# arhix52/Strelka

Measured on AMD Instinct MI355X. Metric: Mray/s, higher is better.
Workload: dtype f32; 1 GPU; kitchen stand-in (SURVEY 8d C3): 1724134 unique triangles, 2022 instances of 153 meshes, 4 rect + 1 distant light, 60/25/10/5 % diffuse/glossy/metal/glass; resolution=1920x1080, bounces=4, spp=64, tile=32, world_size=1, parallelism=single GPU, rays_per_frame=839862650

## Files before the change

### strelka_amd/build.py

```python
import os
import subprocess

HERE = os.path.dirname(os.path.abspath(__file__))
ROOT = os.path.dirname(HERE)
LIB = os.environ.get("SKH_LIB") or os.path.join(HERE, "libstrelka_hip.so")
SRC = os.path.join(HERE, "csrc", "strelka_hip.hip")
DEPS = [SRC] + [os.path.join(HERE, "csrc", f) for f in ("skh_device.h", "skh_bvh.h", "skh_env.h", "skh_emit.h", "skh_blend.h", "skh_lshape.h", "skh_kernels.h", "skh_shade_body.inc", "skh_trace_body.inc", "skh_libm.h", "skh_host.h", "skh_accel.inc")] + [
    os.path.join(ROOT, "include", "strelka_hip.h"), os.path.abspath(__file__)]
FLAGS = ["-O3", "--offload-arch=gfx950", "-ffp-contract=off", "-fno-slp-vectorize", "-mllvm", "-amdgpu-sched-strategy=max-ilp",
         "-fPIC", "-shared", "-std=c++17"]


def hipcc():
    for c in (os.environ.get("HIPCC"), "/opt/rocm/bin/hipcc", "hipcc"):
        if c and (os.path.isabs(c) and os.path.exists(c) or not os.path.isabs(c)):
            return c
    return "hipcc"


def needs_build():
    if os.environ.get("SKH_LIB") and os.path.exists(LIB):
        return False
    return not os.path.exists(LIB) or any(os.path.getmtime(d) > os.path.getmtime(LIB) for d in DEPS)


def build_variant(out_path, defines, verbose=False):
    cmd = [hipcc()] + FLAGS + ["-D" + d for d in defines] + ["-o", out_path, SRC]
    if verbose:
        print(" ".join(cmd))
    subprocess.check_call(cmd)
    return out_path


def build(force=False, verbose=False):
    if not force and not needs_build():
        return LIB
    import fcntl

    with open(LIB + ".lock", "w") as lock:
        fcntl.flock(lock, fcntl.LOCK_EX)
# ... 60 lines not shown
```

### strelka_amd/csrc/skh_host.h

```cpp
#pragma once
#include "../../include/strelka_hip.h"
#include "skh_kernels.h"

#include <string>
#include <utility>
#include <vector>

typedef struct ncclComm* ncclComm_t;
using namespace skh;

namespace
{
struct DevBuf
{
    void* p = nullptr;
    size_t bytes = 0;
    DevBuf() = default;
    DevBuf(const DevBuf&) = delete;
    DevBuf& operator=(const DevBuf&) = delete;
    DevBuf(DevBuf&& o) noexcept : p(o.p), bytes(o.bytes)
    {
        o.p = nullptr;
        o.bytes = 0;
    }
    DevBuf& operator=(DevBuf&& o) noexcept
    {
        if (this != &o)
        {
            reset();
            p = o.p, bytes = o.bytes;
            o.p = nullptr, o.bytes = 0;
        }
        return *this;
    }
    ~DevBuf()
// ... 139 lines not shown
    uint32_t width = 0, height = 0, tileSize = 32, tileShift = 5, numTiles = 0, numSlots = 0;
    std::vector<uint32_t> tileXY;
    bool customTiles = false;
    DevBuf dTileXY, dAccum, dDiffuse, dSpecular, dDiffCnt, dSpecCnt, dSums, dPath, dRayQ[2], dHits, dShadowQ, dContrib, dCounts,
        dOvf, dOvf2, dStats, dScratchImage;
    uint32_t traceBlocks = 0;
    uint32_t curveSplitBuilt = 1;
    uint32_t numWorldCurves = 0;
    int worldCurveRoot[SKH_WORLD_CURVES];
    uint32_t worldCurveInst[SKH_WORLD_CURVES];
    uint32_t worldCurveMerged = 0;
    uint32_t worldCurveIdentLast = 0;
    uint32_t hierNodes = 0;
    int32_t fetchChunk = -1;
    uint32_t numTlasLeaves = 0;
    bool countTraversal = false, timing = false;
    uint32_t wavesPerCU = 28;
    uint32_t wavesPerCUShadow = 28;
    uint32_t wavesPerCUShadowWorld = 32;
    uint32_t queueConstBits[2] = { 0, 0 };
    bool queueConstFilled = false;
    uint32_t reinsertRounds = 8;
    uint32_t reinsertCurveRounds = 4;
    uint32_t reinsertMinSize = 0;
    skh_build_info buildInfo = {};
    uint32_t plocTop = 0;
    uint32_t wavesPerCUWorld = 32;
    uint32_t smallWavesClosest = 0, smallWavesShadow = 0;
    uint32_t gridOverride = 0;
    uint32_t fetchMinClosestSmall = 48;
    bool fetchMinClosestSet = false;
    uint32_t smallWavesFirst = 0, smallWavesLast = 0;
    int tailSplit = 1;
    bool splitNow = false;
    uint32_t fetchMinClosest = 32 , fetchMinShadow = 48;
    uint32_t curveFetchMinClosest = 16, curveFetchMinShadow = 16 , curveNodeBreakClosest = 20, curveNodeBreakShadow = 20;
    uint32_t nodeBreakClosest = 32, nodeBreakShadow = 28;
    uint32_t worldCurveMin = 32;
    uint32_t curveMin = 48;
    uint32_t leafMin = 16;
    uint32_t subframeBatch = 0, batchCapacity = 1;
    uint32_t queueRegion = 64;
    bool tightInstanceBoxes = true;
    uint32_t curveLeaf = 1;
    uint32_t numMergedCurveInst = 0;
    uint32_t splitPairs = 0;
    uint32_t curveMerge = 1;
    uint32_t curveSegNode = 0;
    uint32_t curveStrandMajor = 0;
    uint32_t curveSplit = 4;
    uint32_t tlasBuild = 1;
    uint32_t tlasOpen = 1;
    uint32_t bakeWorld = 4, bakeSmallTris = 64, bakeBudgetMTris = 64;
    bool worldKernel = true;
    std::vector<uint8_t> baked;
    int worldRoot = SKH_REF_INVALID, lightRoot = SKH_REF_INVALID;
    uint32_t nBakedTris = 0, nBakedInst = 0;
    uint32_t mortonBits = 10;
    uint32_t leafLines = 0;
    uint32_t nTriSlots = 0;
    LightBox lightBox = { { -INFINITY, -INFINITY, -INFINITY }, { INFINITY, INFINITY, INFINITY } };
    uint32_t mergeLightProxies = 0;
    uint32_t nShadeRecords = 0;
    int32_t directRecordsOpt = -1;
    uint32_t directRecords = 1;
    uint32_t hitPrimRange = 0;
// ... 54 lines not shown
```

### strelka_amd/csrc/skh_kernels.h

```cpp
#pragma once
#include "skh_bvh.h"
#include "skh_env.h"
#include "skh_emit.h"
#include "skh_blend.h"

namespace skh
{

struct DevInstance
{
    float w2o[12];
    int rootRef;
    uint32_t mask;
    uint32_t type;
    uint32_t pad;
};
struct HostInstance
{
    float o2w[12];
    uint32_t type, geom, material, light;
};

#define SKH_WORLD_CURVES 2
#define SKH_SEG_STRIDE 8
// ... 119 lines not shown
    return mk3(rcp_safe(d.x), rcp_safe(d.y), rcp_safe(d.z));
}
#define SKH_SLAB_SLACK 1.0000019073486328125f

struct TraceCounters
{
    uint32_t nodes, prims, segs, insts;
};

SKH_DI bool slab_test(const v3& lo, const v3& hi, const v3& o, const v3& inv, float tmin, float tmax, float& tnear)
{
    const float t0x = (lo.x - o.x) * inv.x, t1x = (hi.x - o.x) * inv.x;
    const float t0y = (lo.y - o.y) * inv.y, t1y = (hi.y - o.y) * inv.y;
    const float t0z = (lo.z - o.z) * inv.z, t1z = (hi.z - o.z) * inv.z;
    const float tn = fmaxf(fmaxf(fminf(t0x, t1x), fminf(t0y, t1y)), fmaxf(fminf(t0z, t1z), tmin));
    const float tf = fminf(fminf(fmaxf(t0x, t1x), fmaxf(t0y, t1y)), fminf(fmaxf(t0z, t1z), tmax));
    tnear = tn;
    return tn <= tf * 1.0000002384185791015625f;
}

struct HitRec
{
    float t;
    uint32_t inst, prim;
    float u, v;
    bool found;
};

struct StatsDev
{
    unsigned long long raysRadiance, raysShadow, nodes[2], prims[2], segs[2], insts[2];
#ifdef SKH_LANE_PROFILE
    unsigned long long wave[2][10];
    unsigned long long shade[8];
    unsigned int slowCount, slowPad;
    float slow[16][12];
    unsigned long long runHist[2][42], blockHist[2][42];
    unsigned long long cyc[2][10];
#endif
#ifdef SKH_TAIL_PROFILE
    unsigned long long launchT0[2], dryHist[2][64], exitHist[2][64], afterDryHist[2][64], dryLive[2][65], rayTicksAfterDry[2], waveTicksAfterDry[2];
#endif
};

SKH_DI uint32_t rank_below(unsigned long long mask)
{
    return __builtin_amdgcn_mbcnt_hi((uint32_t)(mask >> 32), __builtin_amdgcn_mbcnt_lo((uint32_t)mask, 0u));
}
SKH_DI uint32_t wave_max(uint32_t v)
{
#pragma unroll
    for (int off = 32; off >= 1; off >>= 1)
        v = max(v, (uint32_t)__shfl_xor(v, off));
    return v;
}

SKH_DI uint32_t wave_sum(uint32_t v)
{
#pragma unroll
    for (int off = 32; off >= 1; off >>= 1)
        v += __shfl_xor(v, off);
    return v;
}

#ifndef SKH_CURVE_MIN_WAVES
#define SKH_CURVE_MIN_WAVES 6
#endif
// ... 611 lines not shown
    if (i >= n)
        return;
    const uint32_t mid0 = material[i] == 0xffffffffu ? 0u : material[i], mid = mid0 < numMaterials ? mid0 : 0u;
    Material mat = materials[mid];
    const float4 l = Le[mid];
    v3 le = mk3(l.x, l.y, l.z);
    resolve_material(texels, texDesc, numTextures, mat, mtex_entry(mt, mid), le, uv[2 * (size_t)i], uv[2 * (size_t)i + 1]);
    float* o = out + 8 * (size_t)i;
    o[0] = mat.base_color[0], o[1] = mat.base_color[1], o[2] = mat.base_color[2], o[3] = mat.roughness, o[4] = mat.metallic;
    o[5] = le.x, o[6] = le.y, o[7] = le.z;
}
__global__ void __launch_bounds__(256) k_emit_probe_mtex(EmitP em, MtexP mt, DevScene sc, const float* __restrict__ in, uint32_t n, uint32_t* __restrict__ out)
{
    const uint32_t i = blockIdx.x * blockDim.x + threadIdx.x;
    if (i >= n)
        return;
    const float* q = in + 6 * (size_t)i;
    const EmitSample s = emit_sample(em, q[0], q[1], q[2], mk3(q[3], q[4], q[5]));
    const v3 Le = s.Le * emit_sample_texel(mt, sc, s.instance, s.prim, q[1], q[2]);
    uint32_t* o = out + 13 * (size_t)i;
    o[0] = __float_as_uint(s.point.x), o[1] = __float_as_uint(s.point.y), o[2] = __float_as_uint(s.point.z);
    o[3] = __float_as_uint(s.normal.x), o[4] = __float_as_uint(s.normal.y), o[5] = __float_as_uint(s.normal.z);
    o[6] = __float_as_uint(Le.x), o[7] = __float_as_uint(Le.y), o[8] = __float_as_uint(Le.z);
    o[9] = __float_as_uint(s.pdf), o[10] = __float_as_uint(s.dist), o[11] = s.instance, o[12] = s.prim;
}

#ifndef SKH_SHADE_WAVES
#define SKH_SHADE_WAVES(HAIR) ((HAIR) ? 4 : 5)
#endif
#define SKH_SHADE_ATTR(HAIR) __attribute__((amdgpu_waves_per_eu(SKH_SHADE_WAVES(HAIR), SKH_SHADE_WAVES(HAIR))))
#ifndef SKH_SHADE_BLOCK
#define SKH_SHADE_BLOCK 256
#endif
template <bool HAIR, bool ENV, bool EMIT, bool MTEX>
__global__ void __launch_bounds__(SKH_SHADE_BLOCK) SKH_SHADE_ATTR(HAIR)
    k_shade(DevScene sc, FrameP fp, uint32_t sampleOffset, uint32_t depth , const uint32_t* __restrict__ tileXY, RayQ rq,
            const uint32_t* __restrict__ countPtr, HitQ hq, PathS ps, RayQ nextQ, uint32_t* __restrict__ nextCount, RayQ shadowQ,
            float4* __restrict__ contrib, uint32_t* __restrict__ shadowCount, EnvP env, EmitP emit, MtexP mtex)
{
    constexpr bool LSHAPE = false;
    const LshapeP lsh = { nullptr };
#include "skh_shade_body.inc"
}
template <bool HAIR, bool ENV, bool EMIT, bool MTEX>
__global__ void __launch_bounds__(SKH_SHADE_BLOCK) SKH_SHADE_ATTR(HAIR)
    k_shade_lshape(DevScene sc, FrameP fp, uint32_t sampleOffset, uint32_t depth , const uint32_t* __restrict__ tileXY, RayQ rq,
                   const uint32_t* __restrict__ countPtr, HitQ hq, PathS ps, RayQ nextQ, uint32_t* __restrict__ nextCount, RayQ shadowQ,
                   float4* __restrict__ contrib, uint32_t* __restrict__ shadowCount, EnvP env, EmitP emit, MtexP mtex, LshapeP lsh)
{
    constexpr bool LSHAPE = true;
#include "skh_shade_body.inc"
}

__global__ void __launch_bounds__(256) k_lshape_probe(const Light* __restrict__ lights, uint32_t numLights, LshapeP lsh, uint32_t rectMethod, uint32_t kind,
                                                      const uint32_t* __restrict__ in, uint32_t n, float* __restrict__ out)
{
    const uint32_t i = blockIdx.x * blockDim.x + threadIdx.x;
    if (i >= n)
        return;
    const uint32_t* q = in + (kind == 0u ? 6u : 7u) * (size_t)i;
    const uint32_t lid = q[0];
    float* o = out + (kind == 0u ? 13u : 2u) * (size_t)i;
    if (lid >= numLights)
    {
        for (uint32_t k = 0; k < (kind == 0u ? 13u : 2u); ++k)
            o[k] = 0.0f;
        return;
    }
    const Light light = lights[lid];
    Lshape lse;
    lse.flags = 0u, lse.cosOuter = lse.cosInner = lse.focus = 0.0f, lse.axis = mk3(0.0f);
    if (lsh.table)
        lse = lshape_fetch(lsh, lid);
    const bool sampledDisc = light.type == 1 && (lse.flags & SKH_LSHAPE_SAMPLE_DISC) != 0u;
    if (kind == 0u)
    {
        const float ux = __uint_as_float(q[1]), uy = __uint_as_float(q[2]);
        const v3 P = mk3(__uint_as_float(q[3]), __uint_as_float(q[4]), __uint_as_float(q[5]));
        LightSample d;
        d.pointOnLight = mk3(0.0f), d.pdf = 0.0f, d.normal = mk3(0.0f), d.area = 0.0f, d.L = mk3(0.0f), d.distToLight = 0.0f;
        switch (light.type)
// ... 682 lines not shown
```

### strelka_amd/csrc/skh_shade_body.inc

```
    const uint32_t numPick = (ENV ? sc.numLights + (env.nee ? 1u : 0u) : sc.numLights) + (EMIT ? (emit.nee ? 1u : 0u) : 0u);
    __shared__ uint32_t s_wave[2 * (SKH_COMPACT_MAX_WAVES + 1)];
    __shared__ uint32_t s_sobol[SKH_SOBOL_LUT_WORDS];
#if SKH_MATERIALS_LDS
    __shared__ float4 s_mat[SKH_MATERIALS_LDS * 4];
#endif
    const uint32_t shard = blockIdx.x & (SKH_SHARDS - 1u), lb = blockIdx.x / SKH_SHARDS;
    const uint32_t n = countPtr[shard * SKH_COUNT_STRIDE];
    if (lb * blockDim.x >= n)
        return;
    const uint32_t il = lb * blockDim.x + threadIdx.x;
    const uint32_t i = shard * rq.region + il;
#ifdef SKH_LANE_PROFILE
    unsigned long long spc[8] = { 0, 0, 0, 0, 0, 0, 0, 0 }, spT = __builtin_readcyclecounter();
#define SKH_SP(k)                                                    \
    {                                                                \
        const unsigned long long t_ = __builtin_readcyclecounter();  \
        spc[k] += t_ - spT;                                          \
        spT = t_;                                                    \
    }
#else
#define SKH_SP(k)
#endif
    bool valid = il < n;
    uint32_t pid = 0;
    v3 rayO = mk3(0.0f), rayD = mk3(0.0f);
    float4 hr0 = make_float4(0.0f, 0.0f, 0.0f, 0.0f), hr1 = hr0;
    {
        constexpr int passes = ((SKH_SOBOL_LUT_WORDS / 4) + SKH_SHADE_BLOCK - 1) / SKH_SHADE_BLOCK;
        uint4 lut[passes];
#pragma unroll
        for (int k = 0; k < passes; ++k)
            if ((k + 1) * SKH_SHADE_BLOCK <= SKH_SOBOL_LUT_WORDS / 4 || threadIdx.x + k * SKH_SHADE_BLOCK < SKH_SOBOL_LUT_WORDS / 4)
                lut[k] = reinterpret_cast<const uint4*>(g_sobol_lut)[threadIdx.x + k * SKH_SHADE_BLOCK];
            else
                lut[k] = make_uint4(0u, 0u, 0u, 0u);
#if SKH_MATERIALS_LDS
        float4 mrow = make_float4(0.0f, 0.0f, 0.0f, 0.0f);
        static_assert(SKH_MATERIALS_LDS * 4 <= SKH_SHADE_BLOCK, "one float4 of the material table per thread");
        if (threadIdx.x < SKH_MATERIALS_LDS * 4 && threadIdx.x < sc.numMaterials * 4u)
            mrow = reinterpret_cast<const float4*>(sc.materials)[threadIdx.x];
#endif
#pragma unroll
        for (int k = 0; k < passes; ++k)
            if ((k + 1) * SKH_SHADE_BLOCK <= SKH_SOBOL_LUT_WORDS / 4 || threadIdx.x + k * SKH_SHADE_BLOCK < SKH_SOBOL_LUT_WORDS / 4)
                reinterpret_cast<uint4*>(s_sobol)[threadIdx.x + k * SKH_SHADE_BLOCK] = lut[k];
#if SKH_MATERIALS_LDS
        if (threadIdx.x < SKH_MATERIALS_LDS * 4)
            s_mat[threadIdx.x] = mrow;
#endif
    }
    __syncthreads();
    bool emitNext = false, emitShadow = false;
    v3 nextO = mk3(0.0f), nextD = mk3(0.0f), shO = mk3(0.0f), shD = mk3(0.0f), shC = mk3(0.0f);
    float shTmax = 0.0f;
    if (valid)
    {
        pid = rq.ids()[i];
        rayO = mk3(rq.plane(0)[i], rq.plane(1)[i], rq.plane(2)[i]);
        rayD = mk3(rq.plane(3)[i], rq.plane(4)[i], rq.plane(5)[i]);
        if (hq.primBits != 0u)
        {
            hr0 = *hq.rec16(i);
            const uint32_t w = __float_as_uint(hr0.w);
            hr1.x = __uint_as_float(w == 0xffffffffu ? w : w >> hq.primBits);
            hr1.y = __uint_as_float(w == 0xffffffffu ? w : ((w & ((1u << hq.primBits) - 1u)) | (hq.direct ? SKH_PRIM_DIRECT : 0u)));
        }
        else
            hr0 = hq.rec(i)[0], hr1 = hq.rec(i)[1];
        const float ht = hr0.x, hu = hr0.y, hv = hr0.z;
        const uint32_t hinst = __float_as_uint(hr1.x), hprim = __float_as_uint(hr1.y);
        float* P = ps.base;
        const size_t S = ps.stride;
        v3 throughput = depth == 0u ? mk3(1.0f) : mk3(P[pid], P[pid + S], P[pid + 2 * S]);
        v3 radiance = mk3(0.0f);
        bool radianceDirty = false;
#define SKH_RADIANCE_LOAD() radiance = mk3(ps.rad()[pid]), radianceDirty = true
        float lastBsdfPdf = depth == 0u ? 0.0f : P[pid + 6 * S];
        uint32_t flags = depth == 0u ? 0u : reinterpret_cast<uint32_t*>(P)[pid + 7 * S];
        bool inside = (flags & PF_INSIDE) != 0;
        bool specularBounce = (flags & PF_SPECULAR) != 0;
        uint32_t firstEvent = (flags >> PF_EVENT_SHIFT) & 3u;
        uint32_t px, py;
        const uint32_t sub = pid / fp.numSlots;
        slot_to_pixel(fp, tileXY, pid - sub * fp.numSlots, px, py);
        Sampler smp = init_sampler(px, py, fp.subframeIndex + sampleOffset + sub, fp.sppTotal, 52u);
        smp.depth = depth;
        uint32_t prdDepth = depth;
        v3 origin = rayO, dir = rayD;

        if (hinst == 0xffffffffu)
        {
            if constexpr (ENV)
            {
                const EnvEval ee = env_eval(env, rayD);
                SKH_RADIANCE_LOAD();
                if (depth == 0 || specularBounce || !env.nee)
                    radiance = radiance + throughput * ee.Le;
                else
                {
                    const float lightPdf = ee.pdf / (float)numPick;
                    const float misWeight = mis_weight_balance(lastBsdfPdf, lightPdf);
// ... 366 lines not shown
        {
            const float p = fmaxf(throughput.x, fmaxf(throughput.y, throughput.z));
            if (sampler_random_lut(smp, DIM_RR, s_sobol) > p)
                alive = false;
            else
                throughput = throughput * (1.0f / (p + 1e-5f));
        }
        if (alive && dot(throughput, throughput) < 1e-5f)
            alive = false;
        if (alive)
        {
            ++prdDepth;
            if (fp.debug == 1)
                alive = false;
        }
        if (alive && prdDepth >= fp.maxDepth)
            alive = false;
        emitNext = alive;
        nextO = origin;
        nextD = dir;
        P[pid] = throughput.x;
        P[pid + S] = throughput.y;
        P[pid + 2 * S] = throughput.z;
        if (radianceDirty)
        {
            ps.rad()[pid] = make_float4(radiance.x, radiance.y, radiance.z, 0.0f);
        }
#undef SKH_RADIANCE_LOAD
        P[pid + 6 * S] = lastBsdfPdf;
        reinterpret_cast<uint32_t*>(P)[pid + 7 * S] =
            (inside ? PF_INSIDE : 0u) | (specularBounce ? PF_SPECULAR : 0u) | (firstEvent << PF_EVENT_SHIFT);
    }
    SKH_SP(6)
    uint32_t ni, si;
    block_compact2(emitNext, nextCount + shard * SKH_COUNT_STRIDE, emitShadow, shadowCount + shard * SKH_COUNT_STRIDE, s_wave, ni, si);
    ni += shard * nextQ.region;
    si += shard * shadowQ.region;
    if (emitNext)
    {
        nextQ.plane(0)[ni] = nextO.x;
        nextQ.plane(1)[ni] = nextO.y;
        nextQ.plane(2)[ni] = nextO.z;
        nextQ.plane(3)[ni] = nextD.x;
        nextQ.plane(4)[ni] = nextD.y;
        nextQ.plane(5)[ni] = nextD.z;
        nextQ.ids()[ni] = pid;
    }
    if (emitShadow)
    {
        shadowQ.plane(0)[si] = shO.x;
        shadowQ.plane(1)[si] = shO.y;
        shadowQ.plane(2)[si] = shO.z;
        shadowQ.plane(3)[si] = shD.x;
        shadowQ.plane(4)[si] = shD.y;
        shadowQ.plane(5)[si] = shD.z;
        shadowQ.plane(7)[si] = shTmax;
        contrib[si] = make_float4(shC.x, shC.y, shC.z, __uint_as_float(pid));
    }
#ifdef SKH_LANE_PROFILE
    SKH_SP(7)
    for (int k = 0; k < 8; ++k)
    {
        const uint32_t hi32 = wave_max((uint32_t)(spc[k] >> 4));
        if ((threadIdx.x & 63u) == 0)
            atomicAdd(&sc.profile->shade[k], (unsigned long long)hi32 << 4);
    }
#endif
#undef SKH_SP
```

### strelka_amd/csrc/strelka_hip.hip

```cpp
#include "../../include/strelka_hip.h"
#include "skh_kernels.h"

#include <dlfcn.h>
typedef struct ncclComm* ncclComm_t;
typedef struct
{
    char internal[128];
} ncclUniqueId;
typedef enum
{
    ncclSuccess = 0
} ncclResult_t;
typedef enum
{
    ncclFloat = 7
} ncclDataType_t;

#include <algorithm>
#include <chrono>
#include <cmath>
#include <cstdio>
#include <cstring>
#include <mutex>
#include <string>
// ... 1600 lines not shown
    const bool oneSampleDirect = batch == 1 && fp.samplesThisLaunch == 1 && finalize && fp.finalFirst == 0 && fp.finalCount == 1;
    for (uint32_t s = 0; trace && s < fp.samplesThisLaunch; ++s)
    {
        SKH_TRY(c, hipMemsetAsync(counts, 0, sizeof(uint32_t) * (QW * 2 * SKH_MAX_LAUNCH_ROUNDS + 16 * SKH_FETCH_STRIDE * (rounds + 1) + (size_t)(cutOn ? rounds : 0u) * cutBounceWords), st));
        blp.sampleBase = fp.subframeIndex + s;
        {
            SpanGuard g(c, KC_RAYGEN);
            k_raygen<<<c->raygenBlocksPerSub * fp.batch, 512, 0, st>>>(fp, tiles, s, rq[0], counts, ps, c->dRaygenBase.as<uint32_t>(),
                                                                       c->raygenBlocksPerSub, c->raygenValidPerSub);
        }
        for (uint32_t b = 0; b < rounds; ++b)
        {
            {
                SpanGuard g(c, KC_TRACE_CLOSEST);
                c->gridOverride = (useOverlap && smallPass) ? ((b == 0 && c->smallWavesFirst) ? c->smallWavesFirst : c->smallWavesClosest ? c->smallWavesClosest : (c->nSegs ? 16u : 20u)) * (uint32_t)c->numCUs : 0u;
                if (c->countTraversal)
                    launch_trace<false, true>(c, sc, rq[b & 1], counts + 2 * b * QW, fetch + 16 * b * SKH_FETCH_STRIDE, hq, ps, nullptr);
                else
                    launch_trace<false, false>(c, sc, rq[b & 1], counts + 2 * b * QW, fetch + 16 * b * SKH_FETCH_STRIDE, hq, ps, nullptr);
                if (cutOn)
                {
                    blp.depth = b;
                    if (c->countTraversal)
                        run_cutout_chain<false, true>(c, sc, sc, rq[b & 1], counts + 2 * b * QW, hq, hq, nullptr, ps, nullptr, cutQ[0], cutQ[1], cutH, cutWords + (size_t)b * cutBounceWords, NP, st, blp);
                    else
                        run_cutout_chain<false, false>(c, sc, sc, rq[b & 1], counts + 2 * b * QW, hq, hq, nullptr, ps, nullptr, cutQ[0], cutQ[1], cutH, cutWords + (size_t)b * cutBounceWords, NP, st, blp);
                }
            }
            if (useOverlap && b > 0)
                (void)hipStreamWaitEvent(st, c->evShadow, 0);
            {
                SpanGuard g(c, KC_SHADE);
                const uint32_t perShard = (((NP + SKH_SHARDS - 1u) / SKH_SHARDS) + 63u) & ~63u;
                const dim3 sg(SKH_SHARDS * ((perShard + SKH_SHADE_BLOCK - 1) / SKH_SHADE_BLOCK));
#define SKH_SHADE_LAUNCH_MTEX(HAIRB, ENVB, EMITB, MTEXB)                                                                                                                             \
    if (lshp.table)                                                                                                                                                                  \
        k_shade_lshape<HAIRB, ENVB, EMITB, MTEXB><<<sg, SKH_SHADE_BLOCK, 0, st>>>(sc, fp, s, b, tiles, rq[b & 1], counts + 2 * b * QW, hq, ps, rq[(b + 1) & 1],                       \
                                                                                  counts + 2 * (b + 1) * QW, shq, c->dContrib.as<float4>(), counts + (2 * b + 1) * QW, envp, emitp,  \
                                                                                  mtexp, lshp);                                                                                      \
    else                                                                                                                                                                             \
        k_shade<HAIRB, ENVB, EMITB, MTEXB><<<sg, SKH_SHADE_BLOCK, 0, st>>>(sc, fp, s, b, tiles, rq[b & 1], counts + 2 * b * QW, hq, ps, rq[(b + 1) & 1], counts + 2 * (b + 1) * QW, \
                                                                           shq, c->dContrib.as<float4>(), counts + (2 * b + 1) * QW, envp, emitp, mtexp)
#define SKH_SHADE_LAUNCH(HAIRB, ENVB, EMITB)              \
    if (mtexp.count)                                      \
    {                                                     \
        SKH_SHADE_LAUNCH_MTEX(HAIRB, ENVB, EMITB, true);  \
    }                                                     \
    else                                                  \
    {                                                     \
        SKH_SHADE_LAUNCH_MTEX(HAIRB, ENVB, EMITB, false); \
    }
#define SKH_SHADE_LAUNCH_EMIT(HAIRB, ENVB)     \
    if (emitp.count)                           \
    {                                          \
        SKH_SHADE_LAUNCH(HAIRB, ENVB, true);   \
    }                                          \
    else                                       \
    {                                          \
        SKH_SHADE_LAUNCH(HAIRB, ENVB, false);  \
    }
                if (c->hasHairMaterial && c->envW)
                {
                    SKH_SHADE_LAUNCH_EMIT(true, true);
                }
                else if (c->hasHairMaterial)
                {
                    SKH_SHADE_LAUNCH_EMIT(true, false);
                }
                else if (c->envW)
                {
                    SKH_SHADE_LAUNCH_EMIT(false, true);
                }
                else
                {
                    SKH_SHADE_LAUNCH_EMIT(false, false);
// ... 1082 lines not shown
struct OptRow
{
    const char* name;
    int64_t lo, hi;
    OptEffect effect;
    void (*store)(skh_context*, int64_t);
    bool needsSegNode = false;
    bool skh_context::*counters = nullptr;
};
static const int64_t kOptMin = INT64_MIN, kOptMax = INT64_MAX;
#define OPT_U32(field) [](skh_context* c, int64_t v) { c->field = (uint32_t)v; }
#define OPT_I32(field) [](skh_context* c, int64_t v) { c->field = (int32_t)v; }
#define OPT_FLAG(field) [](skh_context* c, int64_t v) { c->field = v != 0; }
static const OptRow kOptions[] = {
    { "count_traversal", kOptMin, kOptMax, OPT_NONE, OPT_FLAG(countTraversal), false, &skh_context::countTraversal },
    { "timing", kOptMin, kOptMax, OPT_NONE, OPT_FLAG(timing), false, &skh_context::timing },
    { "fetch_min_closest", 1, 64, OPT_NONE, [](skh_context* c, int64_t v) { c->fetchMinClosestSet = true, c->fetchMinClosest = c->curveFetchMinClosest = (uint32_t)v; } },
    { "fetch_min_shadow", 1, 64, OPT_NONE, [](skh_context* c, int64_t v) { c->fetchMinShadow = c->curveFetchMinShadow = (uint32_t)v; } },
    { "node_break_closest", 0, 64, OPT_NONE, [](skh_context* c, int64_t v) { c->nodeBreakClosest = c->curveNodeBreakClosest = (uint32_t)v; } },
    { "node_break_shadow", 0, 64, OPT_NONE, [](skh_context* c, int64_t v) { c->nodeBreakShadow = c->curveNodeBreakShadow = (uint32_t)v; } },
    { "curve_min", 1, 64, OPT_NONE, [](skh_context* c, int64_t v) { c->curveMin = c->worldCurveMin = (uint32_t)v; } },
    { "fetch_min_closest_small", 1, 64, OPT_NONE, OPT_U32(fetchMinClosestSmall) },
    { "fetch_chunk", -1, 4096, OPT_NONE, OPT_I32(fetchChunk) },
    { "leaf_min", 0, 64, OPT_NONE, OPT_U32(leafMin) },
    { "overlap", 0, 2, OPT_NONE, OPT_I32(overlap) },
    { "tail_split", -1, 2, OPT_NONE, OPT_I32(tailSplit) },
    { "small_waves_first", 0, 64, OPT_NONE, OPT_U32(smallWavesFirst) },
    { "small_waves_last", 0, 64, OPT_NONE, OPT_U32(smallWavesLast) },
    { "small_waves_closest", 0, 64, OPT_NONE, OPT_U32(smallWavesClosest) },
    { "small_waves_shadow", 0, 64, OPT_NONE, OPT_U32(smallWavesShadow) },
    { "env_nee", 0, 1, OPT_NONE, OPT_U32(envNee) },
    { "emit_nee", 0, 1, OPT_NONE, OPT_U32(emitNee) },
    { "cutout_rounds", 1, 32, OPT_NONE, OPT_U32(cutoutRounds) },
    { "speculate", 0, 64, OPT_NONE, OPT_U32(speculateMax) },
    { "speculate_grow", 2, 64, OPT_NONE, OPT_U32(speculateGrow) },
    { "speculate_async", 0, 1, OPT_NONE, [](skh_context* c, int64_t v) { spec_drop(c), c->speculateAsync = (uint32_t)v; } },
    { "world_kernel", kOptMin, kOptMax, OPT_NONE, OPT_FLAG(worldKernel) },
    { "subframe_batch", 0, 64, OPT_FRAME, OPT_U32(subframeBatch) },
    { "waves_per_cu", 1, 32, OPT_FRAME, OPT_U32(wavesPerCU) },
    { "waves_per_cu_shadow", 1, 32, OPT_FRAME, OPT_U32(wavesPerCUShadow) },
    { "waves_per_cu_world", 1, 32, OPT_FRAME, OPT_U32(wavesPerCUWorld) },
    { "waves_per_cu_shadow_world", 1, 32, OPT_FRAME, OPT_U32(wavesPerCUShadowWorld) },
    { "compact_hits", 0, 1, OPT_REBUILD, OPT_U32(compactHits) },
    { "direct_records", -1, 1, OPT_REBUILD, OPT_I32(directRecordsOpt) },
    { "merge_light_proxies", 0, 1, OPT_REBUILD, OPT_U32(mergeLightProxies) },
    { "tight_instance_boxes", kOptMin, kOptMax, OPT_REBUILD, OPT_FLAG(tightInstanceBoxes) },
    { "curve_leaf", 1, 4, OPT_REBUILD, OPT_U32(curveLeaf) },
    { "split_pairs", 0, 1000, OPT_REBUILD, OPT_U32(splitPairs) },
    { "curve_merge", 0, 1, OPT_REBUILD, OPT_U32(curveMerge) },
    { "curve_segnode", 0, 1, OPT_REBUILD, OPT_U32(curveSegNode), true },
    { "curve_strand_major", 0, 1, OPT_REBUILD, OPT_U32(curveStrandMajor), true },
    { "curve_split", 1, 8, OPT_REBUILD, OPT_U32(curveSplit) },
    { "tlas_build", 0, 2, OPT_REBUILD, OPT_U32(tlasBuild) },
    { "tlas_open", 0, 64, OPT_REBUILD, OPT_U32(tlasOpen) },
    { "bake_world", 0, 4, OPT_REBUILD, OPT_U32(bakeWorld) },
    { "bake_budget_mtris", 0, 100, OPT_REBUILD, OPT_U32(bakeBudgetMTris) },
    { "bake_small_tris", 0, 1 << 20, OPT_REBUILD, OPT_U32(bakeSmallTris) },
    { "morton_bits", 4, 21, OPT_REBUILD, OPT_U32(mortonBits) },
    { "leaf_lines", 0, 1, OPT_REBUILD, OPT_U32(leafLines) },
    { "leaf_max_tris", 1, 8, OPT_REBUILD, OPT_U32(leafMaxTris) },
    { "build_quality", kOptMin, kOptMax, OPT_REBUILD, OPT_FLAG(buildQuality) },
    { "reinsert_rounds", 0, 64, OPT_REBUILD, OPT_U32(reinsertRounds) },
    { "reinsert_curve_rounds", 0, 64, OPT_REBUILD, OPT_U32(reinsertCurveRounds) },
    { "reinsert_min_size", 0, 1 << 24, OPT_REBUILD, OPT_U32(reinsertMinSize) },
    { "ploc_top", 0, kOptMax, OPT_REBUILD, OPT_U32(plocTop) },
};
// ... 65 lines not shown
    SKH_TRY(c, hipMemcpy(&sd, c->dStats.p, sizeof(sd), hipMemcpyDeviceToHost));
    memset(out, 0, sizeof(*out));
    uint64_t outR = c->discardedRadiance, outS = c->discardedShadow;
    {
        const skh_context::Speculation& sp = c->spec;
        if (sp.valid && sp.consumed < sp.count && sp.count > 0)
        {
            outR += sp.passRadiance * (sp.count - sp.consumed) / sp.count;
            outS += sp.passShadow * (sp.count - sp.consumed) / sp.count;
        }
        if (sp.nextInFlight)
        {
            outR += sd.raysRadiance - std::min<uint64_t>(sd.raysRadiance, sp.statsMark[0]);
            outS += sd.raysShadow - std::min<uint64_t>(sd.raysShadow, sp.statsMark[1]);
        }
    }
    out->rays_radiance = sd.raysRadiance - std::min<uint64_t>(sd.raysRadiance, outR);
    out->rays_shadow = sd.raysShadow - std::min<uint64_t>(sd.raysShadow, outS);
    out->speculated_discarded = c->discardedSubframes;
    for (int k = 0; k < 2; ++k)
    {
        out->nodes_visited[k] = sd.nodes[k];
        out->prims_tested[k] = sd.prims[k];
        out->segs_tested[k] = sd.segs[k];
        out->instances_entered[k] = sd.insts[k];
    }
#ifdef SKH_LANE_PROFILE
    for (int k = 0; k < 2; ++k)
        fprintf(stderr, "[lane-profile] %s: rays %llu nodes %llu (TLAS %llu) tris %llu insts %llu | wave: nodeIt %llu triIt %llu instBlk %llu outer %llu refills %llu refilled %llu | tri passes with: fp64 fallback %llu, sign test passed %llu, division %llu | curve blocks %llu (instBlk = Newton runs in the curve builds)\n",
                k ? "shadow" : "closest", k ? sd.raysShadow : sd.raysRadiance, sd.nodes[k], sd.segs[k], sd.prims[k], sd.insts[k], sd.wave[k][0], sd.wave[k][1],
                sd.wave[k][2], sd.wave[k][3], sd.wave[k][4], sd.wave[k][5], sd.wave[k][6], sd.wave[k][8], sd.wave[k][7], sd.wave[k][9]);
    {
        double tot = 0;
        for (int k = 0; k < 8; ++k)
            tot += (double)sd.shade[k];
        fprintf(stderr, "[shade-cycles] load %.1f%% hit+material %.1f%% bsdf_sample %.1f%% light %.1f%% bsdf_eval %.1f%% rest-of-hit %.1f%% tail+state %.1f%% compaction+queues %.1f%%\n",
                100 * sd.shade[0] / tot, 100 * sd.shade[1] / tot, 100 * sd.shade[2] / tot, 100 * sd.shade[3] / tot, 100 * sd.shade[4] / tot, 100 * sd.shade[5] / tot,
                100 * sd.shade[6] / tot, 100 * sd.shade[7] / tot);
    }
    fprintf(stderr, "[slow-rays] %u rays took more than 1500 node steps\n", sd.slowCount);
    for (uint32_t k = 0; k < std::min(sd.slowCount, 16u); ++k)
        fprintf(stderr, "[slow-ray] steps %.0f tris %.0f insts %.0f %s o %.9g %.9g %.9g d %.9g %.9g %.9g tmin %g tmax %g\n", sd.slow[k][0], sd.slow[k][1], sd.slow[k][2],
                sd.slow[k][3] != 0.0f ? "shadow" : "closest", sd.slow[k][4], sd.slow[k][5], sd.slow[k][6], sd.slow[k][7], sd.slow[k][8], sd.slow[k][9], sd.slow[k][10], sd.slow[k][11]);
    for (int k = 0; k < 2; ++k)
    {
        unsigned long long tr = 0, tb = 0;
        for (int j = 0; j < 42; ++j)
            tr += sd.runHist[k][j], tb += sd.blockHist[k][j];
        if (tr)
        {
            fprintf(stderr, "[newton-steps] %s runs %llu:", k ? "shadow" : "closest", tr);
            for (int j = 0; j < 42; ++j)
                fprintf(stderr, " %d:%.2f%%", j, 100.0 * (double)sd.runHist[k][j] / (double)tr);
            fprintf(stderr, "\n[newton-block-max] %s rounds %llu:", k ? "shadow" : "closest", tb);
            for (int j = 0; j < 42; ++j)
                fprintf(stderr, " %d:%.2f%%", j, 100.0 * (double)sd.blockHist[k][j] / (double)tb);
            fprintf(stderr, "\n");
        }
    }
    for (int k = 0; k < 2; ++k)
        fprintf(stderr, "[lane-cycles] %s: refill %.3g curve-block %.3g node %.3g leaf %.3g pop %.3g write %.3g total %.3g | shader clock while the waves ran: %.1f MHz (wave-seconds %.4g)\n", k ? "shadow" : "closest", (double)sd.cyc[k][0], (double)sd.cyc[k][8],
                (double)sd.cyc[k][1], (double)sd.cyc[k][2], (double)sd.cyc[k][3], (double)sd.cyc[k][4], (double)sd.cyc[k][5],
                sd.cyc[k][7] ? (double)sd.cyc[k][6] / (double)sd.cyc[k][7] * 100.0 : 0.0, (double)sd.cyc[k][7] / 1e8);
#endif
#ifdef SKH_TAIL_PROFILE
    for (int k = 0; k < 2; ++k)
    {
        unsigned long long waves = 0;
        double liveSum = 0;
        for (int j = 0; j < 64; ++j)
// ... 65 lines not shown
```

Measured before the change: 6395 Mray/s.

## Add optional persistent shade kernel with next-chunk ray/hit prefetch

Packs the shade kernel arguments into one ShadeArgs struct and adds a PERSIST template variant in which a grid sized to CUs times waves loops over ray chunks. It prefetches the next chunk's pid, ray and hit record before compaction, and double-buffers the compaction LDS so consecutive trips do not collide. In persistent mode kernel arguments are re-read from the kernarg segment on each trip to limit register pressure. The default shade_blocks=-1 keeps the non-persistent launch, but the ray and hit loads are still hoisted into registers ahead of the main body, which adds some register pressure to the default path.

```diff
diff --git a/strelka_amd/build.py b/strelka_amd/build.py
--- a/strelka_amd/build.py
+++ b/strelka_amd/build.py
@@ -5,7 +5,7 @@
 ROOT = os.path.dirname(HERE)
 LIB = os.environ.get("SKH_LIB") or os.path.join(HERE, "libstrelka_hip.so")
 SRC = os.path.join(HERE, "csrc", "strelka_hip.hip")
-DEPS = [SRC] + [os.path.join(HERE, "csrc", f) for f in ("skh_device.h", "skh_bvh.h", "skh_env.h", "skh_emit.h", "skh_blend.h", "skh_lshape.h", "skh_kernels.h", "skh_shade_body.inc", "skh_trace_body.inc", "skh_libm.h", "skh_host.h", "skh_accel.inc")] + [
+DEPS = [SRC] + [os.path.join(HERE, "csrc", f) for f in ("skh_device.h", "skh_bvh.h", "skh_env.h", "skh_emit.h", "skh_blend.h", "skh_lshape.h", "skh_kernels.h", "skh_shade_body.inc", "skh_shade_grid.h", "skh_trace_body.inc", "skh_libm.h", "skh_host.h", "skh_accel.inc")] + [
     os.path.join(ROOT, "include", "strelka_hip.h"), os.path.abspath(__file__)]
 FLAGS = ["-O3", "--offload-arch=gfx950", "-ffp-contract=off", "-fno-slp-vectorize", "-mllvm", "-amdgpu-sched-strategy=max-ilp",
          "-fPIC", "-shared", "-std=c++17"]
diff --git a/strelka_amd/csrc/skh_host.h b/strelka_amd/csrc/skh_host.h
--- a/strelka_amd/csrc/skh_host.h
+++ b/strelka_amd/csrc/skh_host.h
@@ -1,6 +1,7 @@
 #pragma once
 #include "../../include/strelka_hip.h"
 #include "skh_kernels.h"
+#include "skh_shade_grid.h"
 
 #include <string>
 #include <utility>
@@ -206,6 +207,7 @@
     bool fetchMinClosestSet = false;
     uint32_t smallWavesFirst = 0, smallWavesLast = 0;
     int tailSplit = 1;
+    int32_t shadeBlocks = -1;
     bool splitNow = false;
     uint32_t fetchMinClosest = 32 , fetchMinShadow = 48;
     uint32_t curveFetchMinClosest = 16, curveFetchMinShadow = 16 , curveNodeBreakClosest = 20, curveNodeBreakShadow = 20;
diff --git a/strelka_amd/csrc/skh_kernels.h b/strelka_amd/csrc/skh_kernels.h
--- a/strelka_amd/csrc/skh_kernels.h
+++ b/strelka_amd/csrc/skh_kernels.h
@@ -175,7 +175,7 @@
     unsigned long long raysRadiance, raysShadow, nodes[2], prims[2], segs[2], insts[2];
 #ifdef SKH_LANE_PROFILE
     unsigned long long wave[2][10];
-    unsigned long long shade[8];
+    unsigned long long shade[9];
     unsigned int slowCount, slowPad;
     float slow[16][12];
     unsigned long long runHist[2][42], blockHist[2][42];
@@ -853,21 +853,56 @@
 #ifndef SKH_SHADE_BLOCK
 #define SKH_SHADE_BLOCK 256
 #endif
-template <bool HAIR, bool ENV, bool EMIT, bool MTEX>
-__global__ void __launch_bounds__(SKH_SHADE_BLOCK) SKH_SHADE_ATTR(HAIR)
-    k_shade(DevScene sc, FrameP fp, uint32_t sampleOffset, uint32_t depth , const uint32_t* __restrict__ tileXY, RayQ rq,
-            const uint32_t* __restrict__ countPtr, HitQ hq, PathS ps, RayQ nextQ, uint32_t* __restrict__ nextCount, RayQ shadowQ,
-            float4* __restrict__ contrib, uint32_t* __restrict__ shadowCount, EnvP env, EmitP emit, MtexP mtex)
+#ifndef SKH_SHADE_PREFETCH_RAY
+#define SKH_SHADE_PREFETCH_RAY 1
+#endif
+struct ShadeArgs
+{
+    DevScene sc;
+    FrameP fp;
+    uint32_t sampleOffset, depth ;
+    const uint32_t* tileXY;
+    RayQ rq;
+    const uint32_t* countPtr;
+    HitQ hq;
+    PathS ps;
+    RayQ nextQ;
+    uint32_t* nextCount;
+    RayQ shadowQ;
+    float4* contrib;
+    uint32_t* shadowCount;
+    EnvP env;
+    EmitP emit;
+    MtexP mtex;
+    LshapeP lsh;
+};
+struct alignas(4) KargWord
+{
+    uint32_t w;
+};
+typedef const __attribute__((address_space(4))) KargWord* KargPtr;
+SKH_DI KargPtr skh_karg_segment()
+{
+    KargPtr kp = (KargPtr)__builtin_amdgcn_kernarg_segment_ptr();
+    asm volatile("" : "+s"(kp));
+    return kp;
+}
+template <class T>
+SKH_DI T skh_karg(KargPtr kp, size_t offset)
+{
+    static_assert(alignof(T) >= 4 && sizeof(T) % 4 == 0, "whole words");
+    T t;
+    __builtin_memcpy(&t, kp + offset / 4, sizeof(T));
+    return t;
+}
+template <bool HAIR, bool ENV, bool EMIT, bool MTEX, bool PERSIST>
+__global__ void __launch_bounds__(SKH_SHADE_BLOCK) SKH_SHADE_ATTR(HAIR) k_shade(ShadeArgs args)
 {
     constexpr bool LSHAPE = false;
-    const LshapeP lsh = { nullptr };
 #include "skh_shade_body.inc"
 }
-template <bool HAIR, bool ENV, bool EMIT, bool MTEX>
-__global__ void __launch_bounds__(SKH_SHADE_BLOCK) SKH_SHADE_ATTR(HAIR)
-    k_shade_lshape(DevScene sc, FrameP fp, uint32_t sampleOffset, uint32_t depth , const uint32_t* __restrict__ tileXY, RayQ rq,
-                   const uint32_t* __restrict__ countPtr, HitQ hq, PathS ps, RayQ nextQ, uint32_t* __restrict__ nextCount, RayQ shadowQ,
-                   float4* __restrict__ contrib, uint32_t* __restrict__ shadowCount, EnvP env, EmitP emit, MtexP mtex, LshapeP lsh)
+template <bool HAIR, bool ENV, bool EMIT, bool MTEX, bool PERSIST>
+__global__ void __launch_bounds__(SKH_SHADE_BLOCK) SKH_SHADE_ATTR(HAIR) k_shade_lshape(ShadeArgs args)
 {
     constexpr bool LSHAPE = true;
 #include "skh_shade_body.inc"
diff --git a/strelka_amd/csrc/skh_shade_body.inc b/strelka_amd/csrc/skh_shade_body.inc
--- a/strelka_amd/csrc/skh_shade_body.inc
+++ b/strelka_amd/csrc/skh_shade_body.inc
@@ -1,17 +1,15 @@
-    const uint32_t numPick = (ENV ? sc.numLights + (env.nee ? 1u : 0u) : sc.numLights) + (EMIT ? (emit.nee ? 1u : 0u) : 0u);
-    __shared__ uint32_t s_wave[2 * (SKH_COMPACT_MAX_WAVES + 1)];
+    __shared__ uint32_t s_wave[2 * 2 * (SKH_COMPACT_MAX_WAVES + 1)];
     __shared__ uint32_t s_sobol[SKH_SOBOL_LUT_WORDS];
 #if SKH_MATERIALS_LDS
     __shared__ float4 s_mat[SKH_MATERIALS_LDS * 4];
 #endif
-    const uint32_t shard = blockIdx.x & (SKH_SHARDS - 1u), lb = blockIdx.x / SKH_SHARDS;
-    const uint32_t n = countPtr[shard * SKH_COUNT_STRIDE];
+    const uint32_t shard = blockIdx.x & (SKH_SHARDS - 1u), lbStep = gridDim.x / SKH_SHARDS;
+    uint32_t lb = blockIdx.x / SKH_SHARDS;
+    const uint32_t n = args.countPtr[shard * SKH_COUNT_STRIDE];
     if (lb * blockDim.x >= n)
         return;
-    const uint32_t il = lb * blockDim.x + threadIdx.x;
-    const uint32_t i = shard * rq.region + il;
 #ifdef SKH_LANE_PROFILE
-    unsigned long long spc[8] = { 0, 0, 0, 0, 0, 0, 0, 0 }, spT = __builtin_readcyclecounter();
+    unsigned long long spc[9] = { 0, 0, 0, 0, 0, 0, 0, 0, 0 }, spT = __builtin_readcyclecounter();
 #define SKH_SP(k)                                                    \
     {                                                                \
         const unsigned long long t_ = __builtin_readcyclecounter();  \
@@ -21,11 +19,32 @@
 #else
 #define SKH_SP(k)
 #endif
-    bool valid = il < n;
-    uint32_t pid = 0;
-    v3 rayO = mk3(0.0f), rayD = mk3(0.0f);
-    float4 hr0 = make_float4(0.0f, 0.0f, 0.0f, 0.0f), hr1 = hr0;
-    {
+    uint32_t pfPid;
+    v3 pfO, pfD;
+    float4 pfH0;
+    float pfH1x, pfH1y;
+#define SKH_SHADE_FETCH(LB)                                                                       \
+    {                                                                                             \
+        const uint32_t il_ = (LB) * blockDim.x + threadIdx.x;                                     \
+        pfPid = 0u, pfO = pfD = mk3(0.0f), pfH0 = make_float4(0.0f, 0.0f, 0.0f, 0.0f);            \
+        pfH1x = pfH1y = 0.0f;                                                                     \
+        if (il_ < n)                                                                              \
+        {                                                                                         \
+            const uint32_t i_ = shard * rq.region + il_;                                          \
+            pfPid = rq.ids()[i_];                                                                 \
+            if (SKH_SHADE_PREFETCH_RAY)                                                           \
+            {                                                                                     \
+                pfO = mk3(rq.plane(0)[i_], rq.plane(1)[i_], rq.plane(2)[i_]);                     \
+                pfD = mk3(rq.plane(3)[i_], rq.plane(4)[i_], rq.plane(5)[i_]);                     \
+            }                                                                                     \
+            if (hq.primBits != 0u)                                                                \
+                pfH0 = *hq.rec16(i_);    \
+            else                                                                                  \
+                pfH0 = hq.rec(i_)[0], pfH1x = hq.rec(i_)[1].x, pfH1y = hq.rec(i_)[1].y;           \
+        }                                                                                         \
+    }
+    {
+        const DevScene& sc = args.sc;
         constexpr int passes = ((SKH_SOBOL_LUT_WORDS / 4) + SKH_SHADE_BLOCK - 1) / SKH_SHADE_BLOCK;
         uint4 lut[passes];
 #pragma unroll
@@ -50,23 +69,58 @@
 #endif
     }
     __syncthreads();
+    SKH_SP(8)
+    {
+        const RayQ rq = args.rq;
+        const HitQ hq = args.hq;
+        SKH_SHADE_FETCH(lb)
+    }
+    for (uint32_t trip = 0;; ++trip)
+    {
+    const KargPtr kp = PERSIST ? skh_karg_segment() : nullptr;
+#define SKH_SHADE_ARG(T, M) const decltype(ShadeArgs::M) M = PERSIST ? skh_karg<decltype(ShadeArgs::M)>(kp, offsetof(ShadeArgs, M)) : args.M
+    SKH_SHADE_ARG(DevScene, sc);
+    SKH_SHADE_ARG(FrameP, fp);
+    SKH_SHADE_ARG(uint32_t, sampleOffset);
+    SKH_SHADE_ARG(uint32_t, depth);
+    SKH_SHADE_ARG(const uint32_t*, tileXY);
+    SKH_SHADE_ARG(RayQ, rq);
+    SKH_SHADE_ARG(HitQ, hq);
+    SKH_SHADE_ARG(PathS, ps);
+    SKH_SHADE_ARG(RayQ, nextQ);
+    SKH_SHADE_ARG(uint32_t*, nextCount);
+    SKH_SHADE_ARG(RayQ, shadowQ);
+    SKH_SHADE_ARG(float4*, contrib);
+    SKH_SHADE_ARG(uint32_t*, shadowCount);
+    SKH_SHADE_ARG(EnvP, env);
+    SKH_SHADE_ARG(EmitP, emit);
+    SKH_SHADE_ARG(MtexP, mtex);
+    SKH_SHADE_ARG(LshapeP, lsh);
+#undef SKH_SHADE_ARG
+    const uint32_t numPick = (ENV ? sc.numLights + (env.nee ? 1u : 0u) : sc.numLights) + (EMIT ? (emit.nee ? 1u : 0u) : 0u);
+    const uint32_t il = lb * blockDim.x + threadIdx.x;
+    const bool valid = il < n;
+    uint32_t pid = 0;
     bool emitNext = false, emitShadow = false;
     v3 nextO = mk3(0.0f), nextD = mk3(0.0f), shO = mk3(0.0f), shD = mk3(0.0f), shC = mk3(0.0f);
     float shTmax = 0.0f;
     if (valid)
     {
-        pid = rq.ids()[i];
-        rayO = mk3(rq.plane(0)[i], rq.plane(1)[i], rq.plane(2)[i]);
-        rayD = mk3(rq.plane(3)[i], rq.plane(4)[i], rq.plane(5)[i]);
+        pid = pfPid;
+        v3 rayO = pfO, rayD = pfD;
+        if (!SKH_SHADE_PREFETCH_RAY)
+        {
+            const uint32_t i = shard * rq.region + il;
+            rayO = mk3(rq.plane(0)[i], rq.plane(1)[i], rq.plane(2)[i]);
+            rayD = mk3(rq.plane(3)[i], rq.plane(4)[i], rq.plane(5)[i]);
+        }
+        float4 hr0 = pfH0, hr1 = make_float4(pfH1x, pfH1y, 0.0f, 0.0f);
         if (hq.primBits != 0u)
         {
-            hr0 = *hq.rec16(i);
             const uint32_t w = __float_as_uint(hr0.w);
             hr1.x = __uint_as_float(w == 0xffffffffu ? w : w >> hq.primBits);
             hr1.y = __uint_as_float(w == 0xffffffffu ? w : ((w & ((1u << hq.primBits) - 1u)) | (hq.direct ? SKH_PRIM_DIRECT : 0u)));
         }
-        else
-            hr0 = hq.rec(i)[0], hr1 = hq.rec(i)[1];
         const float ht = hr0.x, hu = hr0.y, hv = hr0.z;
         const uint32_t hinst = __float_as_uint(hr1.x), hprim = __float_as_uint(hr1.y);
         float* P = ps.base;
@@ -499,8 +553,12 @@
             (inside ? PF_INSIDE : 0u) | (specularBounce ? PF_SPECULAR : 0u) | (firstEvent << PF_EVENT_SHIFT);
     }
     SKH_SP(6)
+    const uint32_t lbNext = lb + lbStep;
+    const bool more = lbNext * blockDim.x < n;
+    if (PERSIST)
+        SKH_SHADE_FETCH(lbNext)
     uint32_t ni, si;
-    block_compact2(emitNext, nextCount + shard * SKH_COUNT_STRIDE, emitShadow, shadowCount + shard * SKH_COUNT_STRIDE, s_wave, ni, si);
+    block_compact2(emitNext, nextCount + shard * SKH_COUNT_STRIDE, emitShadow, shadowCount + shard * SKH_COUNT_STRIDE, s_wave + (trip & 1u) * (2 * (SKH_COMPACT_MAX_WAVES + 1)), ni, si);
     ni += shard * nextQ.region;
     si += shard * shadowQ.region;
     if (emitNext)
@@ -524,13 +582,18 @@
         shadowQ.plane(7)[si] = shTmax;
         contrib[si] = make_float4(shC.x, shC.y, shC.z, __uint_as_float(pid));
     }
+    SKH_SP(7)
+    if (!PERSIST || !more)
+        break;
+    lb = lbNext;
+    }
+#undef SKH_SHADE_FETCH
 #ifdef SKH_LANE_PROFILE
-    SKH_SP(7)
-    for (int k = 0; k < 8; ++k)
+    for (int k = 0; k < 9; ++k)
     {
         const uint32_t hi32 = wave_max((uint32_t)(spc[k] >> 4));
         if ((threadIdx.x & 63u) == 0)
-            atomicAdd(&sc.profile->shade[k], (unsigned long long)hi32 << 4);
+            atomicAdd(&args.sc.profile->shade[k], (unsigned long long)hi32 << 4);
     }
 #endif
 #undef SKH_SP
diff --git a/strelka_amd/csrc/skh_shade_grid.h b/strelka_amd/csrc/skh_shade_grid.h
--- /dev/null
+++ b/strelka_amd/csrc/skh_shade_grid.h
@@ -0,0 +1,23 @@
+#pragma once
+#include <cstdint>
+
+namespace skh
+{
+static const int64_t kShadeBlocksMin = -1, kShadeBlocksMax = 65536;
+
+inline uint32_t shade_blocks_round(uint32_t v, uint32_t shards)
+{
+    return (v + shards - 1u) / shards * shards;
+}
+inline int32_t shade_blocks_store(int64_t v, uint32_t shards)
+{
+    return v > 0 ? (int32_t)shade_blocks_round((uint32_t)v, shards) : (int32_t)v;
+}
+inline uint32_t shade_grid(int32_t stored, uint32_t chunkGrid, uint32_t numCUs, uint32_t wgPerCU, uint32_t shards)
+{
+    if (stored < 0)
+        return chunkGrid;
+    const uint32_t want = stored > 0 ? shade_blocks_round((uint32_t)stored, shards) : shade_blocks_round(numCUs * wgPerCU, shards);
+    return want < chunkGrid ? want : chunkGrid;
+}
+}
diff --git a/strelka_amd/csrc/strelka_hip.hip b/strelka_amd/csrc/strelka_hip.hip
--- a/strelka_amd/csrc/strelka_hip.hip
+++ b/strelka_amd/csrc/strelka_hip.hip
@@ -1656,15 +1656,19 @@
             {
                 SpanGuard g(c, KC_SHADE);
                 const uint32_t perShard = (((NP + SKH_SHARDS - 1u) / SKH_SHARDS) + 63u) & ~63u;
-                const dim3 sg(SKH_SHARDS * ((perShard + SKH_SHADE_BLOCK - 1) / SKH_SHADE_BLOCK));
-#define SKH_SHADE_LAUNCH_MTEX(HAIRB, ENVB, EMITB, MTEXB)                                                                                                                             \
-    if (lshp.table)                                                                                                                                                                  \
-        k_shade_lshape<HAIRB, ENVB, EMITB, MTEXB><<<sg, SKH_SHADE_BLOCK, 0, st>>>(sc, fp, s, b, tiles, rq[b & 1], counts + 2 * b * QW, hq, ps, rq[(b + 1) & 1],                       \
-                                                                                  counts + 2 * (b + 1) * QW, shq, c->dContrib.as<float4>(), counts + (2 * b + 1) * QW, envp, emitp,  \
-                                                                                  mtexp, lshp);                                                                                      \
-    else                                                                                                                                                                             \
-        k_shade<HAIRB, ENVB, EMITB, MTEXB><<<sg, SKH_SHADE_BLOCK, 0, st>>>(sc, fp, s, b, tiles, rq[b & 1], counts + 2 * b * QW, hq, ps, rq[(b + 1) & 1], counts + 2 * (b + 1) * QW, \
-                                                                           shq, c->dContrib.as<float4>(), counts + (2 * b + 1) * QW, envp, emitp, mtexp)
+                const dim3 sg(shade_grid(c->shadeBlocks, SKH_SHARDS * ((perShard + SKH_SHADE_BLOCK - 1) / SKH_SHADE_BLOCK), (uint32_t)c->numCUs,
+                                         (uint32_t)SKH_SHADE_WAVES(c->hasHairMaterial) * 256u / SKH_SHADE_BLOCK, SKH_SHARDS));
+                const ShadeArgs sa = { sc, fp, s, b, tiles, rq[b & 1], counts + 2 * b * QW, hq, ps, rq[(b + 1) & 1], counts + 2 * (b + 1) * QW, shq, c->dContrib.as<float4>(),
+                                       counts + (2 * b + 1) * QW, envp, emitp, mtexp, lshp };
+#define SKH_SHADE_LAUNCH_MTEX(HAIRB, ENVB, EMITB, MTEXB)                                       \
+    if (lshp.table && c->shadeBlocks >= 0)                                                     \
+        k_shade_lshape<HAIRB, ENVB, EMITB, MTEXB, true><<<sg, SKH_SHADE_BLOCK, 0, st>>>(sa);   \
+    else if (lshp.table)                                                                       \
+        k_shade_lshape<HAIRB, ENVB, EMITB, MTEXB, false><<<sg, SKH_SHADE_BLOCK, 0, st>>>(sa);  \
+    else if (c->shadeBlocks >= 0)                                                              \
+        k_shade<HAIRB, ENVB, EMITB, MTEXB, true><<<sg, SKH_SHADE_BLOCK, 0, st>>>(sa);          \
+    else                                                                                       \
+        k_shade<HAIRB, ENVB, EMITB, MTEXB, false><<<sg, SKH_SHADE_BLOCK, 0, st>>>(sa)
 #define SKH_SHADE_LAUNCH(HAIRB, ENVB, EMITB)              \
     if (mtexp.count)                                      \
     {                                                     \
@@ -2813,6 +2817,7 @@
     { "env_nee", 0, 1, OPT_NONE, OPT_U32(envNee) },
     { "emit_nee", 0, 1, OPT_NONE, OPT_U32(emitNee) },
     { "cutout_rounds", 1, 32, OPT_NONE, OPT_U32(cutoutRounds) },
+    { "shade_blocks", kShadeBlocksMin, kShadeBlocksMax, OPT_NONE, [](skh_context* c, int64_t v) { c->shadeBlocks = shade_blocks_store(v, SKH_SHARDS); } },
     { "speculate", 0, 64, OPT_NONE, OPT_U32(speculateMax) },
     { "speculate_grow", 2, 64, OPT_NONE, OPT_U32(speculateGrow) },
     { "speculate_async", 0, 1, OPT_NONE, [](skh_context* c, int64_t v) { spec_drop(c), c->speculateAsync = (uint32_t)v; } },
@@ -2944,10 +2949,10 @@
                 sd.wave[k][2], sd.wave[k][3], sd.wave[k][4], sd.wave[k][5], sd.wave[k][6], sd.wave[k][8], sd.wave[k][7], sd.wave[k][9]);
     {
         double tot = 0;
-        for (int k = 0; k < 8; ++k)
+        for (int k = 0; k < 9; ++k)
             tot += (double)sd.shade[k];
-        fprintf(stderr, "[shade-cycles] load %.1f%% hit+material %.1f%% bsdf_sample %.1f%% light %.1f%% bsdf_eval %.1f%% rest-of-hit %.1f%% tail+state %.1f%% compaction+queues %.1f%%\n",
-                100 * sd.shade[0] / tot, 100 * sd.shade[1] / tot, 100 * sd.shade[2] / tot, 100 * sd.shade[3] / tot, 100 * sd.shade[4] / tot, 100 * sd.shade[5] / tot,
+        fprintf(stderr, "[shade-cycles] staging %.1f%% load %.1f%% hit+material %.1f%% bsdf_sample %.1f%% light %.1f%% bsdf_eval %.1f%% rest-of-hit %.1f%% tail+state %.1f%% compaction+queues %.1f%%\n",
+                100 * sd.shade[8] / tot, 100 * sd.shade[0] / tot, 100 * sd.shade[1] / tot, 100 * sd.shade[2] / tot, 100 * sd.shade[3] / tot, 100 * sd.shade[4] / tot, 100 * sd.shade[5] / tot,
                 100 * sd.shade[6] / tot, 100 * sd.shade[7] / tot);
     }
     fprintf(stderr, "[slow-rays] %u rays took more than 1500 node steps\n", sd.slowCount);
```

New measurement: 6393 Mray/s. Within noise of the previous version (-0.0%).
